# zoltanmaric/h264-fer

Hardware: AMD Instinct MI355X
Metric: macroblocks/sec encode (1080p full-search ME) + bit-exact bitstream vs ref (higher is better)
Workload: dtype u8; 1 GPU; 1080p IPPP encode, full-search +-16 ME (BASELINE configs[2]); content=textured, coded_size=1920x1072, streams_per_gpu=256, contexts_per_gpu=1, gop=30, qp=12, window=32, maxdiff=3, parallelism=1 x 256 independent closed-GOP streams

## Files before the change

h264-fer_amd/csrc/fer_me.hip:

```cpp
#include <stdlib.h>
#include "fer_internal.h"
#include "fer_mvpred.h"

#define INF_M 1000000000

struct WList {
    int m;
    int xy;
};

__device__ __forceinline__ int pack_xy(int x, int y) { return (x & 0xffff) | (y << 16); }
__device__ __forceinline__ int unp_x(int xy) { return (int)(short)(xy & 0xffff); }
__device__ __forceinline__ int unp_y(int xy) { return xy >> 16; }

__device__ __forceinline__ void wl_insert(WList &L, int K, int lane, bool valid, int m, int xy)
{
    int thr = lane_bcast(L.m, K - 1);
    unsigned long long mask = __ballot(valid && m < thr);
    while (mask) {
        int src = __ffsll((long long)mask) - 1;
        mask &= mask - 1;
        int cm = lane_bcast(m, src), cxy = lane_bcast(xy, src);
        int pos = __popcll(__ballot(lane < K && L.m <= cm));
        if (pos < K) {
// ... 164 lines not shown
    select_topk_ex<NB, true>(v, K, lane, sel, L, raw, fin, [&](int u) { return u * 64 + lane; });
}

typedef unsigned short u16x2_t __attribute__((ext_vector_type(2)));
typedef short i16x2_t __attribute__((ext_vector_type(2)));
__device__ __forceinline__ uint32_t pk_sub16(uint32_t a, uint32_t b)
{
    return __builtin_bit_cast(uint32_t, (u16x2_t)(__builtin_bit_cast(u16x2_t, a) - __builtin_bit_cast(u16x2_t, b)));
}
__device__ __forceinline__ uint32_t pk_abs16(uint32_t a)
{
    i16x2_t x = __builtin_bit_cast(i16x2_t, a), z = {0, 0};
    return __builtin_bit_cast(uint32_t, __builtin_elementwise_max(x, (i16x2_t)(z - x)));
}
struct SuPk {
    uint32_t s01, s23, s4;
    uint32_t d01, d23, d4;
    uint32_t s12, s34;
    uint32_t e12, e34;
};
__device__ __forceinline__ SuPk su_pack(const int s[5])
{
    SuPk p;
    p.s01 = (uint32_t)s[0] | ((uint32_t)s[1] << 16);
    p.s23 = (uint32_t)s[2] | ((uint32_t)s[3] << 16);
    p.s4 = (uint32_t)s[4];
    p.d01 = (uint32_t)(s[0] - s[1]) << 16;
    p.d23 = (uint32_t)(s[0] - s[2]) | ((uint32_t)(s[0] - s[3]) << 16);
    p.d4 = (uint32_t)(s[0] - s[4]);
    p.s12 = (uint32_t)s[1] | ((uint32_t)s[2] << 16);
    p.s34 = (uint32_t)s[3] | ((uint32_t)s[4] << 16);
    p.e12 = (uint32_t)(s[0] - s[1]) | ((uint32_t)(s[0] - s[2]) << 16);
    p.e34 = (uint32_t)(s[0] - s[3]) | ((uint32_t)(s[0] - s[4]) << 16);
    return p;
}
__device__ __forceinline__ int feat_dist_w(uint32_t a, uint32_t b, uint32_t c, const SuPk &p)
{
    uint32_t t = __builtin_amdgcn_sad_u16(a, p.s01, 0);
    t = __builtin_amdgcn_sad_u16(b, p.s23, t);
    t = __builtin_amdgcn_sad_u16(c, p.s4, t);
    uint32_t kk = __builtin_amdgcn_perm(a, a, 0x01000100);
    t = __builtin_amdgcn_sad_u16(pk_sub16(kk, a), p.d01, t);
    t = __builtin_amdgcn_sad_u16(pk_sub16(kk, b), p.d23, t);
    t = __builtin_amdgcn_sad_u16(pk_sub16(kk, c) & 0xffffu, p.d4, t);
    return (int)t;
}
__device__ __forceinline__ int feat_dist_rec(const uint16_t *__restrict__ rec, const SuPk &p)
{
    const uint32_t *r = (const uint32_t *)rec;
    return feat_dist_w(r[0], r[1], r[2], p);
}
struct FeatRec {
    uint32_t a, b, c;
};

__device__ __forceinline__ FeatRec feat_rec_direct(const IPlanes &ip, int W, int H, int frac, int refy, int refx)
{
    const int y = iclamp(refy, 0, H - 1), x = iclamp(refx, 0, W - 1);
    const uint8_t *p0 = ip.base + (size_t)frac * ip.plane + (size_t)y * ip.pitch + (x & ~3);
    const uint32_t sh = (uint32_t)(x & 3);
    uint32_t h84[8], hc[8];
#pragma unroll
    for (int r = 0; r < 8; r++) {
        const uint32_t *w = (const uint32_t *)(p0 + (size_t)r * ip.pitch);
        const uint32_t lo = __builtin_amdgcn_alignbyte(w[1], w[0], sh), hi = __builtin_amdgcn_alignbyte(w[2], w[1], sh);
        const uint32_t a4 = __builtin_amdgcn_sad_u8(lo, 0u, 0u);
        h84[r] = __builtin_amdgcn_sad_u8(hi, 0u, a4) | (a4 << 16);
        hc[r] = __builtin_amdgcn_udot4(hi, 0x00000101u, __builtin_amdgcn_udot4(lo, 0x00000101u, 0u, false), false);
    }
    const uint32_t top = h84[0] + h84[1] + h84[2] + h84[3], all = top + h84[4] + h84[5] + h84[6] + h84[7];
    const uint32_t k3 = (h84[0] + h84[1] + h84[4] + h84[5]) & 0xffffu;
    const uint32_t k4 = hc[0] + hc[1] + hc[2] + hc[3] + hc[4] + hc[5] + hc[6] + hc[7];
    FeatRec f;
    f.a = (all & 0xffffu) | (top << 16);
    f.b = (all >> 16) | (k3 << 16);
    f.c = k4;
    return f;
}

template <int R1>
struct LocalGeo {
    static constexpr int N1 = 2 * R1 + 1, PW = 2 * R1 + 8, NC = N1 * N1 * 16, NB = (NC + 63) / 64;
    static constexpr int HTAB = 8 * PW * N1 * 2;
};
template <int R1>
struct LocalLoads {
    static constexpr int ROUNDS = (8 * LocalGeo<R1>::PW + 63) / 64;
    uint4 w[2][ROUNDS];
};
template <int R1>
__device__ __forceinline__ void local_request(const IPlanes &ip, int W, int H, int px0, int py0, int lane, LocalLoads<R1> &ld)
{
    using G = LocalGeo<R1>;
    constexpr int N1 = G::N1, PW = G::PW;
#pragma unroll
    for (int half = 0; half < 2; half++)
#pragma unroll
        for (int k = 0; k < LocalLoads<R1>::ROUNDS; k++) ld.w[half][k] = make_uint4(0, 0, 0, 0);
    if (px0 + N1 - 1 < 0 || px0 >= W || py0 + N1 - 1 < 0 || py0 >= H) return;
    const uint8_t *mbase = ip.base - ((size_t)FER_IP_T * ip.pitch + FER_IP_L);
    const uint32_t obase = __umul24((uint32_t)(py0 + FER_IP_T), (uint32_t)ip.pitch) + (uint32_t)((px0 & ~3) + FER_IP_L);
#pragma unroll
    for (int half = 0; half < 2; half++) {
#pragma unroll
        for (int k = 0; k < LocalLoads<R1>::ROUNDS; k++) {
            const int tt = min(k * 64 + lane, 8 * PW - 1);
            const int fl = tt / PW, r = tt - fl * PW;
            typedef uint32_t u32x4_a4 __attribute__((ext_vector_type(4), aligned(4)));
            const u32x4_a4 v = *(const u32x4_a4 *)(mbase + (obase + __umul24((uint32_t)(half * 8 + fl), (uint32_t)ip.plane) + __umul24((uint32_t)r, (uint32_t)ip.pitch)));
            ld.w[half][k] = make_uint4(v.x, v.y, v.z, v.w);
        }
    }
}
template <int R1>
__device__ __forceinline__ void local_metrics(const IPlanes &ip, int W, int H, int px0, int py0, const SuPk &sp, int lane,
                                              uint32_t *htab, int *mtab, int half_lo = 0, int half_hi = 2, const LocalLoads<R1> *pre = nullptr)
{
    using G = LocalGeo<R1>;
    constexpr int N1 = G::N1, PW = G::PW;
    static_assert(PW + 3 <= 16, "the patch row must fit one 16-byte load");
    if (px0 + N1 - 1 < 0 || px0 >= W || py0 + N1 - 1 < 0 || py0 >= H) {
#pragma unroll
        for (int u = 0; u < G::NB; u++) mtab[u * 64 + lane] = -1;
        WAVE_LDS_SYNC();
        return;
    }
    const uint32_t sh = (uint32_t)(px0 & 3);
    const uint8_t *mbase = ip.base - ((size_t)FER_IP_T * ip.pitch + FER_IP_L);
    const uint32_t obase = __umul24((uint32_t)(py0 + FER_IP_T), (uint32_t)ip.pitch) + (uint32_t)((px0 & ~3) + FER_IP_L);
    for (int half = half_lo; half < half_hi; half++) {
#pragma unroll
        for (int t0 = 0; t0 < 8 * PW; t0 += 64) {
            const int t = t0 + lane;
            const int tt = min(t, 8 * PW - 1);
            const int fl = tt / PW, r = tt - fl * PW;
            typedef uint32_t u32x4_a4 __attribute__((ext_vector_type(4), aligned(4)));
            uint4 w;
            if (pre) {
                w = half == 0 ? pre->w[0][t0 / 64] : pre->w[1][t0 / 64];
            } else {
                const u32x4_a4 v = *(const u32x4_a4 *)(mbase + (obase + __umul24((uint32_t)(half * 8 + fl), (uint32_t)ip.plane) + __umul24((uint32_t)r, (uint32_t)ip.pitch)));
                w = make_uint4(v.x, v.y, v.z, v.w);
            }
            const uint32_t b0 = __builtin_amdgcn_alignbyte(w.y, w.x, sh), b1 = __builtin_amdgcn_alignbyte(w.z, w.y, sh),
                           b2 = __builtin_amdgcn_alignbyte(w.w, w.z, sh);
            if (t < 8 * PW) {
                uint32_t *o = htab + (size_t)tt * N1 * 2;
#pragma unroll
                for (int ix = 0; ix < N1; ix++) {
                    const uint32_t lo = ix < 4 ? __builtin_amdgcn_alignbyte(b1, b0, (uint32_t)(ix & 3)) : b1;
                    const uint32_t hi = ix < 4 ? __builtin_amdgcn_alignbyte(b2, b1, (uint32_t)(ix & 3)) : b2;
                    const uint32_t a4 = __builtin_amdgcn_sad_u8(lo, 0u, 0u);
                    o[ix * 2] = __builtin_amdgcn_sad_u8(hi, 0u, a4) | (a4 << 16);
                    o[ix * 2 + 1] = __builtin_amdgcn_udot4(hi, 0x00000101u, __builtin_amdgcn_udot4(lo, 0x00000101u, 0u, false), false);
                }
            }
        }
        WAVE_LDS_SYNC();
        if (lane < 8 * N1) {
            const int fl = lane / N1, ix = lane - fl * N1;
            uint32_t P84[PW + 1], Pc[PW + 1];
            P84[0] = 0;
            Pc[0] = 0;
#pragma unroll
            for (int r = 0; r < PW; r++) {
                const uint2 h = *(const uint2 *)(htab + ((size_t)(fl * PW + r) * N1 + ix) * 2);
                P84[r + 1] = P84[r] + h.x;
                Pc[r + 1] = Pc[r] + h.y;
            }
            const int refx = px0 + ix, wx = iabs(ix - R1) + 4;
            const bool xok = refx >= 0 && refx < W;
#pragma unroll
            for (int iy = 0; iy < N1; iy++) {
                const uint32_t all = P84[iy + 8] - P84[iy];
                const uint32_t k1 = (P84[iy + 4] - P84[iy]) & 0xffffu;
                const uint32_t k3 = ((P84[iy + 2] - P84[iy]) + (P84[iy + 6] - P84[iy + 4])) & 0xffffu;
                const uint32_t k4 = Pc[iy + 8] - Pc[iy];
                const int D = feat_dist_w((all & 0xffffu) | (k1 << 16), (all >> 16) | (k3 << 16), k4, sp);
                const int refy = py0 + iy;
                const int m = (int)__umul24((uint32_t)(wx + iabs(iy - R1)), (uint32_t)D) | ((xok && refy >= 0 && refy < H) ? 0 : -1);
                mtab[((ix * N1 + iy) << 4) + half * 8 + fl] = m;
            }
        }
        WAVE_LDS_SYNC();
    }
    if (half_lo == 0) {
#pragma unroll
        for (int c = G::NC + lane; c < G::NB * 64; c += 64) mtab[c] = -1;
    }
    WAVE_LDS_SYNC();
}

__device__ __forceinline__ FeatRec feat0_load(const uint16_t *__restrict__ F0, int W, int H, int refy, int refx)
{
    int y = iclamp(refy, 0, H - 1), x = iclamp(refx, 0, W - 1);
    const uint32_t *r = (const uint32_t *)((const char *)F0 + (__umul24((uint32_t)y, (uint32_t)W * 12u) + (uint32_t)x * 12u));
    FeatRec f;
    f.a = r[0];
    f.b = r[1];
    f.c = r[2];
    return f;
}

struct SrcBlk {
    uint32_t lo[8], hi[8];
};
__device__ __forceinline__ SrcBlk src_block_load(const uint8_t *__restrict__ Y, int W, int sx, int sy)
{
    SrcBlk b;
#pragma unroll
    for (int r = 0; r < 8; r++) {
        const uint32_t *q = (const uint32_t *)(Y + (size_t)(sy + r) * W + sx);
        b.lo[r] = __builtin_amdgcn_readfirstlane((int)q[0]);
        b.hi[r] = __builtin_amdgcn_readfirstlane((int)q[1]);
    }
    return b;
}
__device__ __forceinline__ int sad_lane(const IPlanes &ip, int W, int H, int sx, int sy, int mvx, int mvy, const SrcBlk &S)
{
    const int xPi = iclamp(sx + (mvx >> 2), 0, W - 1), yPi = iclamp(sy + (mvy >> 2), 0, H - 1);
    const uint32_t sh = (uint32_t)(xPi & 3);
    const uint32_t o0 = __umul24((uint32_t)((mvx & 3) + (mvy & 3) * 4), (uint32_t)ip.plane) + __umul24((uint32_t)yPi, (uint32_t)ip.pitch) + (uint32_t)(xPi & ~3);
    uint32_t w[8][3];
#pragma unroll
    for (int r = 0; r < 8; r++) {
        const uint32_t *a = (const uint32_t *)(ip.base + (o0 + __umul24((uint32_t)r, (uint32_t)ip.pitch)));
        w[r][0] = a[0];
        w[r][1] = a[1];
        w[r][2] = a[2];
    }
    uint32_t sad = 0;
#pragma unroll
    for (int r = 0; r < 8; r++) {
        const uint32_t r0 = __builtin_amdgcn_alignbyte(w[r][1], w[r][0], sh), r1 = __builtin_amdgcn_alignbyte(w[r][2], w[r][1], sh);
        sad = __builtin_amdgcn_sad_u8(r1, S.hi[r], __builtin_amdgcn_sad_u8(r0, S.lo[r], sad));
    }
    return (int)sad;
}

#define ME_WIDE_LDS 1156
#define ME_SEL_NB 25
#ifndef PRE_WAVES
#define PRE_WAVES 5
#endif
template <int WIN>
__global__ __launch_bounds__(64) __attribute__((amdgpu_waves_per_eu(PRE_WAVES, PRE_WAVES))) void k_me_pre(FerDev d)
{
    const int window = WIN ? WIN : d.window;
    __shared__ __attribute__((aligned(16))) int wide_m[ME_WIDE_LDS];
    __shared__ __attribute__((aligned(16))) int sel_lds[448];
    static_assert(LocalGeo<2>::HTAB <= ME_WIDE_LDS && LocalGeo<2>::NB * 64 <= 448, "LDS regions of k_me_pre");
    const int lane = threadIdx.x;
    const int s = blockIdx.y;
    if (d.hdr[s * 4 + 3] != 0) return;
    const unsigned bx = xcd_swizzle(blockIdx.x, gridDim.x);
    const int mb = (int)(bx >> 2), part = (int)(bx & 3);
    const int W = d.W, H = d.H;
    const size_t ysz = d.ysz;
    const uint8_t *Y = d.curY + (size_t)s * ysz;
    const IPlanes ip = ip_stream(d, s);
    const int sx = ((mb % d.mbw) << 4) + (part & 1) * 8, sy = ((mb / d.mbw) << 4) + (part >> 1) * 8;
    const size_t pidx = ((size_t)s * d.nmb + mb) * 4 + part;

#ifdef FER_PROBE
    const bool probe = FER_DBGF(d, 128) && s == 0 && (bx % 997) == 5;
    long long tmark = probe ? wall_clock64() : 0;
#define PP_MARK(k)                                                          \
    if (probe) {                                                            \
        long long now_ = wall_clock64();                                    \
        if (lane == 0) atomicAdd((unsigned long long *)&d.timing[32 + k], (unsigned long long)(now_ - tmark)); \
        tmark = now_;                                                       \
    }
#else
#define PP_MARK(k)
#endif
    constexpr int RRL = (WIN == 16) ? 1 : 2;
    LocalLoads<RRL> ld;
    const bool fast_path = (WIN == 32 || WIN == 16) && !FER_DBGF(d, 3) && !d.basic;
    if (fast_path) local_request<RRL>(ip, W, H, sx - RRL, sy - RRL, lane, ld);
    int px = lane & 7, py = lane >> 3;
    int v = Y[(size_t)(sy + py) * W + sx + px];
    int su[5];
    su[0] = wave_sum(v);
    su[1] = wave_sum(py > 3 ? 0 : v);
    su[2] = wave_sum(px > 3 ? 0 : v);
    su[3] = wave_sum((py & 3) > 1 ? 0 : v);
    su[4] = wave_sum((px & 3) > 1 ? 0 : v);
    if (lane < 5) d.suma[pidx * 5 + lane] = su[lane];
    if (d.basic) {
        if (lane == 0) {
            d.st3n[pidx] = 0;
            d.v0[pidx] = 0;
        }
        return;
    }
    const SuPk sp = su_pack(su);
    PP_MARK(0)

    WList L;
    L.m = INF_M;
    L.xy = 0;
    const int R = window / 2, n = 2 * R + 1;
    const int r2 = window / 16, n2w = 2 * r2 + 1, nloc = n2w * n2w * 16;
    const uint16_t *F0 = d.feat0 + (size_t)s * 6 * ysz;
    const int wb = (n * n + 63) >> 6;
    if ((WIN == 32 || WIN == 16) && !FER_DBGF(d, 3)) {
        constexpr int WCH = 6;
        constexpr int NN = (WIN ? WIN : 32) + 1;
        constexpr int NBc = WIN ? WIN : 32, RPB = 64 / NBc, NWB = (NN + RPB - 1) / RPB;
        constexpr int LB = LocalGeo<RRL>::NB;
        static_assert(LB <= 7, "ME_SEL_NB leaves room for 7 local batches");
        const int ix = lane % NBc, r0 = lane / NBc;
        const int rx = sx - R + ix;
        const bool xok = rx >= 0 && rx < W;
        const int wx = iabs(ix - R) + 4;
        const uint32_t colo = (uint32_t)iclamp(rx, 0, W - 1) * 12u, rowb = (uint32_t)W * 12u;
        auto fin = [&](int idx) {
            if (idx < wb * 64) return pack_xy((idx / n - R) * 4, (idx % n - R) * 4);
            int c = idx - wb * 64;
            int frac = c & 15, pos = c >> 4;
            return pack_xy((pos / n2w - r2) * 4 + (frac & 3), (pos % n2w - r2) * 4 + (frac >> 2));
        };
        uint32_t k0w[NWB];
#pragma unroll
        for (int b2 = 0; b2 < NWB; b2++) {
            const int ry = iclamp(sy - R + b2 * RPB + r0, 0, H - 1);
            k0w[b2] = *(const uint32_t *)((const char *)F0 + (colo + __umul24((uint32_t)ry, rowb)));
        }
        const uint32_t k0c = feat0_load(F0, W, H, sy - R + min(lane, NN - 1), sx + R).a;
        local_metrics<RRL>(ip, W, H, sx - r2, sy - r2, sp, lane, (uint32_t *)wide_m, sel_lds, 0, 2, &ld);
        int vloc[LB];
        unsigned lminl = 0xffffffffu;
#pragma unroll
        for (int u = 0; u < LB; u++) {
            vloc[u] = sel_lds[u * 64 + lane];
            lminl = min(lminl, (unsigned)vloc[u]);
        }
        int T = 0x7fffffff;
        if (__popcll(__ballot(lminl < (1u << 21))) >= 33) {
            int lo = 0, hi = (1 << 21) - 1;
            while (lo < hi) {
                const int mid = (lo + hi) >> 1;
                if (__popcll(__ballot(lminl <= (unsigned)mid)) >= 33)
                    hi = mid;
                else
                    lo = mid + 1;
            }
            T = lo;
        }
        int *surv = wide_m;
        int ns = 0;
        const uint32_t s0 = (uint32_t)su[0];
        bool done = false;
        if (T != 0x7fffffff) {
#pragma unroll
            for (int b2 = 0; b2 < NWB; b2++) {
                const int iy = b2 * RPB + r0;
                const int ry = sy - R + iy;
                const uint32_t lb = __umul24(5u * (uint32_t)(wx + iabs(iy - R)), __builtin_amdgcn_sad_u16(k0w[b2] & 0xffffu, s0, 0u));
                const bool take = xok && ry >= 0 && ry < H && iy < NN && lb <= (uint32_t)T;
                const unsigned long long mk = __ballot(take);
                if (mk) {
                    const int slot = ns + (int)__builtin_amdgcn_mbcnt_hi((uint32_t)(mk >> 32), __builtin_amdgcn_mbcnt_lo((uint32_t)mk, 0u));
                    if (take && slot < 128) surv[slot] = ix * NN + iy;
                    ns += __popcll(mk);
                }
            }
            {
                const int iy = lane, ry = sy - R + iy;
                const uint32_t lb = __umul24(5u * (uint32_t)(R + 4 + iabs(iy - R)), __builtin_amdgcn_sad_u16(k0c & 0xffffu, s0, 0u));
                const bool take = iy < NN && sx + R < W && ry >= 0 && ry < H && lb <= (uint32_t)T;
                const unsigned long long mk = __ballot(take);
                if (mk) {
                    const int slot = ns + (int)__builtin_amdgcn_mbcnt_hi((uint32_t)(mk >> 32), __builtin_amdgcn_mbcnt_lo((uint32_t)mk, 0u));
                    if (take && slot < 128) surv[slot] = (NN - 1) * NN + iy;
                    ns += __popcll(mk);
                }
            }
            WAVE_LDS_SYNC();
            if (ns <= 128) {
                int v[2 + LB], ar[2];
#pragma unroll
                for (int b2 = 0; b2 < 2; b2++) {
                    v[b2] = -1;
                    ar[b2] = 0;
                    if (b2 * 64 < ns) {
                        const int idx = b2 * 64 + lane;
                        const bool on = idx < ns;
                        const int ai = on ? surv[idx] : 0;
                        const int cix = ai / NN, ciy = ai - cix * NN;
                        const FeatRec f = feat0_load(F0, W, H, sy - R + ciy, sx - R + cix);
                        const int m = (int)__umul24((uint32_t)(iabs(cix - R) + iabs(ciy - R) + 4), (uint32_t)feat_dist_w(f.a, f.b, f.c, sp));
                        v[b2] = on ? m : -1;
                        ar[b2] = ai;
                    }
                }
#pragma unroll
                for (int u = 0; u < LB; u++) v[2 + u] = vloc[u];
                WAVE_LDS_SYNC();
                auto arrv = [&](int u) { return u < 2 ? ar[u < 2 ? u : 0] : wb * 64 + (u - 2) * 64 + lane; };
                done = select_topk_ex<2 + LB, false>(v, 33, lane, sel_lds, L, arrv, fin, arrv);
            }
        }
        PP_MARK(1)
#ifdef FER_STATS
        if (lane == 0) {
            atomicAdd((unsigned long long *)&d.timing[48], 1ull);
            atomicAdd((unsigned long long *)&d.timing[49], done ? 0ull : 1ull);
            atomicAdd((unsigned long long *)&d.timing[50], (unsigned long long)ns);
            atomicAdd((unsigned long long *)&d.timing[51], T == 0x7fffffff ? 1ull : 0ull);
            atomicAdd((unsigned long long *)&d.timing[52], (unsigned long long)(T == 0x7fffffff ? 0 : T));
        }
#endif
        if (!done) {
            WAVE_LDS_SYNC();
            auto wide_load = [&](int iy0, FeatRec (&fr)[WCH]) {
#pragma unroll
                for (int q = 0; q < WCH; q++) {
                    int ry = iclamp(sy - R + iy0 + q * RPB + r0, 0, H - 1);
                    const uint32_t *r = (const uint32_t *)((const char *)F0 + (colo + __umul24((uint32_t)ry, rowb)));
                    fr[q].a = r[0];
                    fr[q].b = r[1];
                    fr[q].c = r[2];
                }
            };
            auto wide_eval = [&](int iy0, const FeatRec (&fr)[WCH]) {
#pragma unroll
                for (int q = 0; q < WCH; q++) {
                    const int iy = iy0 + q * RPB + r0;
                    const int ry = sy - R + iy;
                    const int m = (int)__umul24((uint32_t)(wx + iabs(iy - R)), (uint32_t)feat_dist_w(fr[q].a, fr[q].b, fr[q].c, sp));
                    const int bad = (xok && ry >= 0 && ry < H) ? 0 : -1;
                    wide_m[iy < n ? ix * n + iy : ME_WIDE_LDS - 1] = m | bad;
                }
            };
            {
                constexpr int STEP = RPB * WCH;
                FeatRec fa[WCH], fb[WCH];
                wide_load(0, fa);
                for (int iy0 = 0; iy0 < n; iy0 += 2 * STEP) {
                    if (iy0 + STEP < n) wide_load(iy0 + STEP, fb);
                    wide_eval(iy0, fa);
                    if (iy0 + STEP < n) {
                        if (iy0 + 2 * STEP < n) wide_load(iy0 + 2 * STEP, fa);
                        wide_eval(iy0 + STEP, fb);
                    }
                }
            }
            {
                const int iy = min(lane, n - 1);
                const int rxl = sx + R, ry = sy - R + iy;
                FeatRec f = feat0_load(F0, W, H, ry, rxl);
                int m = (R + 4 + iabs(iy - R)) * feat_dist_w(f.a, f.b, f.c, sp);
                if (!(rxl < W && ry >= 0 && ry < H)) m = -1;
                if (lane < n) wide_m[(n - 1) * n + iy] = m;
            }
            __syncthreads();
            int v[ME_SEL_NB];
#pragma unroll
            for (int u = 0; u < ME_SEL_NB; u++) {
                v[u] = -1;
                if (u < wb) {
                    int c = u * 64 + lane;
                    if (c < n * n) v[u] = wide_m[c];
                } else if (u - wb < LB) {
                    v[u] = vloc[u - wb < LB ? u - wb : 0];
                }
            }
            WAVE_LDS_SYNC();
            auto raw = [&](int u) { return u * 64 + lane; };
            PP_MARK(2)
            select_topk<ME_SEL_NB>(v, 33, lane, sel_lds, L, raw, fin);
        }
        PP_MARK(3)
    } else {
        for (int base = 0; base < n * n && !FER_DBGF(d, 1); base += 64) {
            int c = base + lane;
            int tx = c / n - R, ty = c % n - R;
            int rx = sx + tx, ry = sy + ty;
            bool ok = c < n * n && rx >= 0 && rx < W && ry >= 0 && ry < H;
            int m = 0;
            if (ok) m = (iabs(tx) + iabs(ty) + 4) * feat_dist_rec(F0 + ((size_t)ry * W + rx) * 6, sp);
            wl_insert(L, 33, lane, ok, m, pack_xy(tx * 4, ty * 4));
        }
        for (int base = 0; base < nloc && !FER_DBGF(d, 2); base += 64) {
            int c = base + lane;
            int frac = c & 15, pos = c >> 4;
            int tx = pos / n2w - r2, ty = pos % n2w - r2;
            int rx = sx + tx, ry = sy + ty;
            bool ok = c < nloc && rx >= 0 && rx < W && ry >= 0 && ry < H;
            int m = 0;
            if (ok) {
                const FeatRec f = feat_rec_direct(ip, W, H, frac, ry, rx);
                m = (iabs(tx) + iabs(ty) + 4) * feat_dist_w(f.a, f.b, f.c, sp);
            }
            wl_insert(L, 33, lane, ok, m, pack_xy(tx * 4 + (frac & 3), ty * 4 + (frac >> 2)));
        }
    }
    const int n3 = __popcll(__ballot(lane < 33 && L.m < 100000000));
    int v0 = 0;
    if (!FER_DBGF(d, 4)) {
        const SrcBlk SB = src_block_load(Y, W, sx, sy);
        const int cx = unp_x(L.xy), cy = unp_y(L.xy);
        const int sad = sad_lane(ip, W, H, sx, sy, lane < n3 ? cx : 0, lane < n3 ? cy : 0, SB);
        if (lane < n3) {
            int *o = d.st3 + (pidx * 33 + lane) * 3;
            o[0] = cx;
            o[1] = cy;
            o[2] = sad;
        }
        const int wk = wave_min(lane < n3 ? (sad << 6) | lane : 0x7fffffff);
        if (wk != 0x7fffffff) v0 = lane_bcast(L.xy, wk & 63);
    }
    if (lane == 0) {
        d.st3n[pidx] = n3;
        d.v0[pidx] = v0;
    }

}

struct NoProbe {
    __device__ __forceinline__ int operator()(int) const { return 0; }
};
template <bool QUIRK, class SINK, class PROBE = NoProbe>
__device__ __forceinline__ int walk_buckets_q(const FerDev &d, int s, const int (&su)[5], const SuPk &sp, int sx, int sy, int lane,
                                              uint32_t *tbl, int halt_cnt, int &jend, SINK sink, uint32_t max_slice = 0xffffffffu,
                                              bool skip0 = false, PROBE probe = PROBE())
{
    int tren = 0;
    jend = 180;
    const int kt = d.kt;
    const uint32_t *kol2 = d.kol2 + (size_t)s * 16384 * kt;
    const uint32_t *srec = d.sort_rec;
    const int n0 = QUIRK ? d.zero_cnt[s] : 0;
    const uint32_t npos = (uint32_t)(d.W * d.H), g0 = (uint32_t)s * npos;
    const uint16_t *F0 = d.feat0 + (size_t)s * 6 * d.ysz;
    const int t_lo = QUIRK ? 0 : (max(sx - 279, 0) >> d.ktw_shift), t_hi = QUIRK ? kt - 1 : (min(sx + 279, d.W - 1) >> d.ktw_shift);
    auto qstart = [&](int a) -> uint32_t {
        if (a <= 0) return g0;
        if (a == 1) return g0 + min(2u * (uint32_t)n0, npos);
        if (a >= 16384) return g0 + npos;
        return kol2[(size_t)a * kt] - (uint32_t)n0;
    };
    const uint32_t sxy = ((uint32_t)sx << 16) | (uint32_t)sy;
    const char *srec_s = (const char *)(srec + (size_t)g0 * 3);
    auto fetch = [&](unsigned b_start, int b_cnt, uint32_t &r0, uint32_t &r1, uint32_t &r2) {
        const uint32_t li = (b_start - g0) + (unsigned)min(lane, max(b_cnt - 1, 0));
        const uint32_t *e = (const uint32_t *)(srec_s + __umul24(li, 12u));
        r0 = e[0];
        r1 = e[1];
        r2 = e[2];
    };
    auto passes = [&](uint32_t r0, uint32_t r1) -> bool {
        uint32_t dist = __builtin_amdgcn_sad_u16(r0, sxy, 0);
        uint32_t e12 = pk_abs16(pk_sub16(r1, sp.s12));
        return dist < 280u && (pk_sub16(e12, 0x00640064u) & 0x80008000u) == 0x80008000u;
    };
    auto feat_d = [&](uint32_t info, uint32_t r0, uint32_t r1, uint32_t r2) -> uint32_t {
        uint32_t D;
        if (!QUIRK) {
            const uint32_t aa = ((info >> 16) & 0x7fffu) * 0x10001u;
            D = __builtin_amdgcn_sad_u16(r1, sp.s12, (info >> 8) & 255u);
            D = __builtin_amdgcn_sad_u16(r2, sp.s34, D);
            D = __builtin_amdgcn_sad_u16(pk_sub16(aa, r1), sp.e12, D);
            D = __builtin_amdgcn_sad_u16(pk_sub16(aa, r2), sp.e34, D);
        } else {
            int px = min((int)(r0 >> 16), d.W - 1), py = min((int)(r0 & 0xffff), d.H - 1);
            D = (uint32_t)feat_dist_rec(F0 + ((size_t)py * d.W + px) * 6, sp);
        }
        return D;
    };
    auto filter = [&](uint32_t info, uint32_t r0, uint32_t r1, uint32_t r2) -> bool {
        const int b_cnt = (int)(info & 127u);
        bool ok = lane < b_cnt && passes(r0, r1);
        unsigned long long mk = __ballot(ok);
        int rank = tren + (int)__builtin_amdgcn_mbcnt_hi((uint32_t)(mk >> 32), __builtin_amdgcn_mbcnt_lo((uint32_t)mk, 0u));
        const uint32_t D = feat_d(info, r0, r1, r2);
        const bool halt = sink(ok, rank, (int)pk_sub16(r0, sxy), (int)D, info);
        tren += __popcll(mk);
        return halt || tren > halt_cnt;
    };
    auto run_table = [&](uint32_t dstart, uint32_t dinfo, int nb) -> bool {
        auto desc = [&](int b, unsigned &bs, uint32_t &bi) {
            const int bb = min(b, 63);
            bs = (unsigned)__builtin_amdgcn_readlane((int)dstart, bb);
            bi = (uint32_t)__builtin_amdgcn_readlane((int)dinfo, bb);
        };
        unsigned sA, sB, sC, sD;
        uint32_t iA, iB, iC, iD;
        uint32_t A0, A1, A2, B0, B1, B2, C0, C1, C2, D0, D1, D2;
        desc(0, sA, iA);
        fetch(sA, (int)(iA & 127u), A0, A1, A2);
        desc(1, sB, iB);
        fetch(sB, (int)(iB & 127u), B0, B1, B2);
        desc(2, sC, iC);
        fetch(sC, (int)(iC & 127u), C0, C1, C2);
        desc(3, sD, iD);
        fetch(sD, (int)(iD & 127u), D0, D1, D2);
#define WALK_STEP(SS, II, R0, R1, R2, NEXT)                                  \
        if (filter(II, R0, R1, R2)) {       \
            jend = (int)((II >> 8) & 255u);                                  \
// ... 713 lines not shown
    if (d.basic || FER_DBGF(d, 32)) return 0;
    const uint32_t cfl = (uint32_t)lane_bcast(P.e2[0].y, 41);
    const bool rewalk = (cfl & 0x40000000u) != 0 && ((cfl >> 16) & 15u) == 0;
    if (P.n2raw > FER_ST2_CAP && d.zero_cnt[s] == 0 && !rewalk) {
        resolve_crowded(d, s, sx, sy, lane, P, genx, geny, L2);
    } else if (P.n2raw > FER_ST2_CAP) {
        const SuPk sp = su_pack(P.su);
        int jx;
        walk_buckets(d, s, P.su, sp, sx, sy, lane, (uint32_t *)sel_lds, 0x7fffffff, jx, [&](bool ok, int rank, int rel, int D, uint32_t) {
            (void)rank;
            int tx = rel >> 16, ty = (int)(short)(rel & 0xffff);
            wl_insert(L2, 33, lane, ok, (iabs(tx - genx) + iabs(ty - geny) + 4) * D, pack_xy(tx * 4, ty * 4));
            return false;
        });
    } else {
        int m2[FER_ST2_CAP / 64];
#pragma unroll
        for (int u = 0; u < FER_ST2_CAP / 64; u++) {
            int cc = u * 64 + lane;
            int tx = P.e2[u].x >> 16, ty = (int)(short)(P.e2[u].x & 0xffff);
            m2[u] = (int)__umul24((uint32_t)(iabs(tx - genx) + iabs(ty - geny) + 4), (uint32_t)P.e2[u].y) | (cc < P.n2 ? 0 : -1);
        }
        auto raw2 = [&](int u) { return P.e2[u].x; };
        auto fin2 = [&](int e) { return pack_xy((e >> 16) * 4, (int)(short)(e & 0xffff) * 4); };
        select_topk<FER_ST2_CAP / 64>(m2, 33, lane, sel_lds, L2, raw2, fin2);
    }
    return __popcll(__ballot(lane < 33 && L2.m < 100000000));
}

template <int WIN>
__device__ __forceinline__ void resolve_stage23(const FerDev &d, int s, int gx, int gy, int lane, const ResPre &P, int mvpx, int mvpy,
                                                int *sel_lds, int &k2, int &xy2, int &k3, int &xy3)
{
    k2 = k3 = 0x7fffffff;
    xy2 = xy3 = 0;
    if (d.basic || FER_DBGF(d, 32)) return;
    WList L2;
    const int cnt2 = stage2_list(d, s, gx, gy, lane, P, mvpx >> 2, mvpy >> 2, sel_lds, L2);
    if (FER_DBGF(d, 256)) L2.xy = pack_xy(lane & 7, lane >> 3);
    int b2, b2xy;
    sad_keys<33>(L2, cnt2, lane, ip_stream(d, s), d.W, d.H, gx * 8, gy * 8, P.sb, mvpx, mvpy, b2, b2xy);
    wave_best(b2, b2xy, k2, xy2);
    int key = 0x7fffffff;
    if (lane < P.n3) key = ((P.c3s + iabs(P.c3x - mvpx) + iabs(P.c3y - mvpy)) << 6) | lane;
    wave_best(key, pack_xy(P.c3x, P.c3y), k3, xy3);
}

__device__ __forceinline__ ResNbr nbr_from_field(const FerDev &d, const int *vf, int gx, int gy, int lane)
{
    ResNbr N;
    nbr_avail(gx, gy, d.mbw * 2, N.vB, N.vC, N.vD, N.vC16);
    N.vA = gx > 0;
    const int xa = gx + (lane == 0 ? 0 : (lane == 1 ? 1 : (lane == 2 ? -1 : (lane == 3 ? 2 : -1)))), ya = lane == 4 ? gy : gy - 1;
    const bool val = lane == 0 ? N.vB : (lane == 1 ? N.vC : (lane == 2 ? N.vD : (lane == 3 ? N.vC16 : (lane == 4 && N.vA))));
    const int w = val ? vf[part_slot(d.mbw, xa, ya)] : 0;
    N.B = lane_bcast(w, 0);
    N.C = lane_bcast(w, 1);
    N.D = lane_bcast(w, 2);
    N.C16 = lane_bcast(w, 3);
    N.A = lane_bcast(w, 4);
    return N;
}

#ifndef SPEC_WAVES
#define SPEC_WAVES 7
#endif
template <int WIN>
__global__ __launch_bounds__(256) __attribute__((amdgpu_waves_per_eu(SPEC_WAVES, SPEC_WAVES))) void k_me_spec(FerDev d)
{
    __shared__ __attribute__((aligned(16))) uint32_t loc_all[4][LocalGeo<2>::HTAB + LocalGeo<2>::NB * 64];
    __shared__ int skipflag;
    static_assert(LocalGeo<2>::HTAB >= 256, "the selection's scratch fits the row sums");
    const int lane = threadIdx.x & 63;
    const int part = __builtin_amdgcn_readfirstlane(threadIdx.x >> 6);
    const int s = blockIdx.y;
    if (d.hdr[s * 4 + 3] != 0) return;
    const int mb = (int)xcd_swizzle(blockIdx.x, gridDim.x);
    const int mbx = mb % d.mbw, mby = mb / d.mbw;
    const int gx = mbx * 2 + (part & 1), gy = mby * 2 + (part >> 1);
    const size_t pidx = ((size_t)s * d.nmb + mb) * 4 + part;
    uint32_t *htab = loc_all[part];
    int *mtab = (int *)loc_all[part] + LocalGeo<2>::HTAB;
    int *sel_lds = (int *)loc_all[part];
    const ResNbr N = nbr_from_field(d, d.v0 + (size_t)s * d.nmb * 4, gx, gy, lane);
    int mvpx, mvpy;
    predict_nbr(N.vA, N.A, N.vB, N.B, N.vC, N.C, N.vD, N.D, mvpx, mvpy);
    const int genx = mvpx >> 2, geny = mvpy >> 2;
    const int genw = pack_xy(genx, geny);
    const int W = d.W, H = d.H;
    const IPlanes ip = ip_stream(d, s);
    const int sx = gx * 8, sy = gy * 8;
    constexpr int RRL = (WIN == 16) ? 1 : 2;
    LocalLoads<RRL> ld;
    if (WIN == 32 || WIN == 16) local_request<RRL>(ip, W, H, sx + genx - RRL, sy + geny - RRL, lane, ld);
    ResPre P;
    res_prefetch(d, s, gx, gy, lane, 1, P);
    int smw = 0;
    bool sk = false;
    if (part == 0) {
        int smx, smy;
        pskip_vector(d, mb, mbx, N, smx, smy);
        smw = pack_xy(smx, smy);
        sk = pskip_test(d, s, mbx, mby, lane, smx, smy);
        if (lane == 0) skipflag = sk;
    }
    __syncthreads();
    sk = skipflag != 0;
    if (sk) {
        if (lane == 0) d.spec_hdr[pidx] = make_int4(genw, part == 0 ? (1 << 17) : 0, smw, 1);
        return;
    }
    if (WIN == 32 || WIN == 16) local_metrics<RRL>(ip, W, H, sx + genx - RRL, sy + geny - RRL, su_pack(P.su), lane, htab, mtab, 0, 2, &ld);
    WList L1, L2;
    const int cnt1 = stage1_list<WIN>(d, s, gx, gy, lane, P, genx, geny, sel_lds, mtab, L1);
    const int cnt2 = stage2_list(d, s, gx, gy, lane, P, genx, geny, sel_lds, L2);
    {
        const int xy2 = __shfl(L2.xy, (lane - 17) & 63);
        const bool first = lane < 17;
        const int xy = first ? L1.xy : xy2;
        const bool on = first ? lane < cnt1 : (lane - 17 < cnt2 && lane < 50);
        const int cx = on ? unp_x(xy) : 0, cy = on ? unp_y(xy) : 0;
        const int sad = sad_lane(ip, W, H, sx, sy, cx, cy, P.sb);
        if (on) {
            int2 *o = first ? d.spec_l1 + (pidx * 17 + lane) : d.spec_l2 + (pidx * 33 + (lane - 17));
            *o = make_int2(xy, sad);
        }
    }
    if (lane == 0) d.spec_hdr[pidx] = make_int4(genw, cnt1 | (cnt2 << 8) | (1 << 16) | (part == 0 ? (1 << 17) : 0), smw, 0);
}

#ifndef RES_WIN
#define RES_WIN 16
#endif
#ifndef RES_WAVES
#define RES_WAVES 6
#endif
template <int WIN>
__global__ __launch_bounds__(64) __attribute__((amdgpu_waves_per_eu(RES_WAVES, RES_WAVES))) void k_me_resolve(FerDev d)
{
    __shared__ __attribute__((aligned(16))) uint32_t loc_lds[LocalGeo<2>::HTAB + LocalGeo<2>::NB * 64];
    const int lane = threadIdx.x;
    const int gw = d.mbw * 2, gh = d.mbh * 2;
    int xcc;
    asm volatile("s_getreg_b32 %0, hwreg(HW_REG_XCC_ID)" : "=s"(xcc));
    const int nq = d.S >= 16 ? 8 : 1;
    const int q_own = nq == 8 ? (xcc & 7) : 0;
    int q_done = 0;
    const bool spec = d.speculate != 0;
    unsigned st_parts = 0, st_hits = 0, st_skq = 0, st_skh = 0;
    for (;;) {
    const int qu = (q_own + q_done) & (nq - 1);
    const int nsq = (d.S - qu + nq - 1) / nq;
    int t = 0;
    if (lane == 0) t = atomicAdd(d.chain + qu, 1);
    t = __builtin_amdgcn_readfirstlane(t);
    const int G = min(d.resolve_group, nsq);
    const int grp = t / (gh * G), rr = t - grp * (gh * G);
    const int k0 = grp * G, kn = min(G, nsq - k0);
    if (k0 >= nsq) {
        if (++q_done == nq) break;
        continue;
    }
    const int gy = rr / kn, s = qu + nq * (k0 + (rr - gy * kn));
    if (gy >= gh) continue;
    if (d.hdr[s * 4 + 3] != 0) continue;
    unsigned long long *chw = d.chain64 + (size_t)s * d.nmb * 4;
    int *mbt = d.mb_type + (size_t)s * d.nmb;
    short *mvs = d.mv + (size_t)s * d.nmb * 8;
    const unsigned serial = (unsigned)d.serial & 0x7fffffffu;

#ifdef FER_PROBE
    const bool probe = FER_DBGF(d, 128) && s == 0 && gy == gh / 2;
#define PR_MARK(k)                        \
    if (probe) {                          \
        long long now_ = wall_clock64();  \
        tacc[k] += now_ - tmark;          \
        tmark = now_;                     \
    }
#else
    const bool probe = false;
#define PR_MARK(k)
#endif
    long long tacc[6] = {0, 0, 0, 0, 0, 0}, tmark = 0;
    int prevw = 0;
    bool skip = false, timeout = false;
    unsigned cwl = 0, cwh = 0;
    int wbase = 0;
    const size_t pidx0 = ((size_t)s * d.nmb + (size_t)(gy >> 1) * d.mbw) * 4 + (size_t)(gy & 1) * 2;
    const int4 *row_hdr = d.spec_hdr + pidx0;
    const int2 *row_l1 = d.spec_l1 + pidx0 * 17, *row_l2 = d.spec_l2 + pidx0 * 33;
    const int *row_st3 = d.st3 + pidx0 * 33 * 3, *row_st3n = d.st3n + pidx0;
    for (int gx = 0; gx < gw; gx++) {
        if (probe) tmark = wall_clock64();
        const int part = (gy & 1) * 2 + (gx & 1);
        const int mbx = gx >> 1, mby = gy >> 1;
        const int mb = mby * d.mbw + mbx;
        int ln = lane;
        asm volatile("" : "+v"(ln));
        int4 sh = make_int4(0, 0, 0, 0);
        int2 e1 = make_int2(0, 0), e2 = make_int2(0, 0);
        int c3x = 0, c3y = 0, c3s = 0, n3 = 0;
        if (spec) {
            const unsigned rp = (FER_DBGF(d, 512) ? 0u : (unsigned)((gx >> 1) * 4 + (gx & 1)));
            sh = row_hdr[rp];
            e1 = row_l1[rp * 17u + (unsigned)min(ln, 16)];
            e2 = row_l2[rp * 33u + (unsigned)min(ln, 32)];
            if (!d.basic) {
                const int *c3 = row_st3 + (rp * 33u + (unsigned)min(ln, 32)) * 3u;
                c3x = c3[0];
                c3y = c3[1];
                c3s = c3[2];
// ... 228 lines not shown
```

Before: 21.02 million macroblocks/s.

## Restructure local metric row loads into three shared rounds and drop prefix sums

Measured after the change: 21.35 million macroblocks/s, median of 6. 1.6% higher.

```diff
diff --git a/h264-fer_amd/csrc/fer_me.hip b/h264-fer_amd/csrc/fer_me.hip
--- a/h264-fer_amd/csrc/fer_me.hip
+++ b/h264-fer_amd/csrc/fer_me.hip
@@ -270,43 +270,44 @@
 struct LocalGeo {
     static constexpr int N1 = 2 * R1 + 1, PW = 2 * R1 + 8, NC = N1 * N1 * 16, NB = (NC + 63) / 64;
     static constexpr int HTAB = 8 * PW * N1 * 2;
+    static constexpr int HT = 8 * PW, ROUNDS = (2 * HT + 63) / 64;
 };
 template <int R1>
 struct LocalLoads {
-    static constexpr int ROUNDS = (8 * LocalGeo<R1>::PW + 63) / 64;
-    uint4 w[2][ROUNDS];
+    static constexpr int EARLY = LocalGeo<R1>::ROUNDS - 1;
+    uint4 w[EARLY];
 };
 template <int R1>
+__device__ __forceinline__ uint4 local_row_load(const uint8_t *mbase, uint32_t obase, const IPlanes &ip, int k, int lane)
+{
+    using G = LocalGeo<R1>;
+    const int t = min(k * 64 + lane, 2 * G::HT - 1);
+    const int fl = t / G::PW, r = t - fl * G::PW;
+    typedef uint32_t u32x4_a4 __attribute__((ext_vector_type(4), aligned(4)));
+    const u32x4_a4 v = *(const u32x4_a4 *)(mbase + (obase + __umul24((uint32_t)fl, (uint32_t)ip.plane) + __umul24((uint32_t)r, (uint32_t)ip.pitch)));
+    return make_uint4(v.x, v.y, v.z, v.w);
+}
+template <int R1>
 __device__ __forceinline__ void local_request(const IPlanes &ip, int W, int H, int px0, int py0, int lane, LocalLoads<R1> &ld)
 {
     using G = LocalGeo<R1>;
-    constexpr int N1 = G::N1, PW = G::PW;
-#pragma unroll
-    for (int half = 0; half < 2; half++)
-#pragma unroll
-        for (int k = 0; k < LocalLoads<R1>::ROUNDS; k++) ld.w[half][k] = make_uint4(0, 0, 0, 0);
+    constexpr int N1 = G::N1;
+#pragma unroll
+    for (int k = 0; k < LocalLoads<R1>::EARLY; k++) ld.w[k] = make_uint4(0, 0, 0, 0);
     if (px0 + N1 - 1 < 0 || px0 >= W || py0 + N1 - 1 < 0 || py0 >= H) return;
     const uint8_t *mbase = ip.base - ((size_t)FER_IP_T * ip.pitch + FER_IP_L);
     const uint32_t obase = __umul24((uint32_t)(py0 + FER_IP_T), (uint32_t)ip.pitch) + (uint32_t)((px0 & ~3) + FER_IP_L);
 #pragma unroll
-    for (int half = 0; half < 2; half++) {
-#pragma unroll
-        for (int k = 0; k < LocalLoads<R1>::ROUNDS; k++) {
-            const int tt = min(k * 64 + lane, 8 * PW - 1);
-            const int fl = tt / PW, r = tt - fl * PW;
-            typedef uint32_t u32x4_a4 __attribute__((ext_vector_type(4), aligned(4)));
-            const u32x4_a4 v = *(const u32x4_a4 *)(mbase + (obase + __umul24((uint32_t)(half * 8 + fl), (uint32_t)ip.plane) + __umul24((uint32_t)r, (uint32_t)ip.pitch)));
-            ld.w[half][k] = make_uint4(v.x, v.y, v.z, v.w);
-        }
-    }
+    for (int k = 0; k < LocalLoads<R1>::EARLY; k++) ld.w[k] = local_row_load<R1>(mbase, obase, ip, k, lane);
 }
 template <int R1>
 __device__ __forceinline__ void local_metrics(const IPlanes &ip, int W, int H, int px0, int py0, const SuPk &sp, int lane,
-                                              uint32_t *htab, int *mtab, int half_lo = 0, int half_hi = 2, const LocalLoads<R1> *pre = nullptr)
+                                              uint32_t *htab, int *mtab, const LocalLoads<R1> *pre = nullptr)
 {
     using G = LocalGeo<R1>;
-    constexpr int N1 = G::N1, PW = G::PW;
+    constexpr int N1 = G::N1, PW = G::PW, HT = G::HT, ROUNDS = G::ROUNDS;
     static_assert(PW + 3 <= 16, "the patch row must fit one 16-byte load");
+    static_assert(HT > 64 && HT <= 128 && ROUNDS == 3, "round 0 belongs to the first half, round 2 to the second, round 1 to both");
     if (px0 + N1 - 1 < 0 || px0 >= W || py0 + N1 - 1 < 0 || py0 >= H) {
 #pragma unroll
         for (int u = 0; u < G::NB; u++) mtab[u * 64 + lane] = -1;
@@ -316,66 +317,74 @@
     const uint32_t sh = (uint32_t)(px0 & 3);
     const uint8_t *mbase = ip.base - ((size_t)FER_IP_T * ip.pitch + FER_IP_L);
     const uint32_t obase = __umul24((uint32_t)(py0 + FER_IP_T), (uint32_t)ip.pitch) + (uint32_t)((px0 & ~3) + FER_IP_L);
-    for (int half = half_lo; half < half_hi; half++) {
-#pragma unroll
-        for (int t0 = 0; t0 < 8 * PW; t0 += 64) {
-            const int t = t0 + lane;
-            const int tt = min(t, 8 * PW - 1);
-            const int fl = tt / PW, r = tt - fl * PW;
-            typedef uint32_t u32x4_a4 __attribute__((ext_vector_type(4), aligned(4)));
-            uint4 w;
-            if (pre) {
-                w = half == 0 ? pre->w[0][t0 / 64] : pre->w[1][t0 / 64];
-            } else {
-                const u32x4_a4 v = *(const u32x4_a4 *)(mbase + (obase + __umul24((uint32_t)(half * 8 + fl), (uint32_t)ip.plane) + __umul24((uint32_t)r, (uint32_t)ip.pitch)));
-                w = make_uint4(v.x, v.y, v.z, v.w);
-            }
-            const uint32_t b0 = __builtin_amdgcn_alignbyte(w.y, w.x, sh), b1 = __builtin_amdgcn_alignbyte(w.z, w.y, sh),
-                           b2 = __builtin_amdgcn_alignbyte(w.w, w.z, sh);
-            if (t < 8 * PW) {
-                uint32_t *o = htab + (size_t)tt * N1 * 2;
-#pragma unroll
-                for (int ix = 0; ix < N1; ix++) {
-                    const uint32_t lo = ix < 4 ? __builtin_amdgcn_alignbyte(b1, b0, (uint32_t)(ix & 3)) : b1;
-                    const uint32_t hi = ix < 4 ? __builtin_amdgcn_alignbyte(b2, b1, (uint32_t)(ix & 3)) : b2;
-                    const uint32_t a4 = __builtin_amdgcn_sad_u8(lo, 0u, 0u);
-                    o[ix * 2] = __builtin_amdgcn_sad_u8(hi, 0u, a4) | (a4 << 16);
-                    o[ix * 2 + 1] = __builtin_amdgcn_udot4(hi, 0x00000101u, __builtin_amdgcn_udot4(lo, 0x00000101u, 0u, false), false);
-                }
-            }
-        }
-        WAVE_LDS_SYNC();
+    const uint4 wlast = local_row_load<R1>(mbase, obase, ip, ROUNDS - 1, lane);
+    auto row_sums = [&](int k, uint2 (&e)[N1]) {
+        const uint4 w = k == ROUNDS - 1 ? wlast : (pre ? pre->w[k] : local_row_load<R1>(mbase, obase, ip, k, lane));
+        const uint32_t b0 = __builtin_amdgcn_alignbyte(w.y, w.x, sh), b1 = __builtin_amdgcn_alignbyte(w.z, w.y, sh),
+                       b2 = __builtin_amdgcn_alignbyte(w.w, w.z, sh);
+#pragma unroll
+        for (int ix = 0; ix < N1; ix++) {
+            const uint32_t lo = ix < 4 ? __builtin_amdgcn_alignbyte(b1, b0, (uint32_t)(ix & 3)) : b1;
+            const uint32_t hi = ix < 4 ? __builtin_amdgcn_alignbyte(b2, b1, (uint32_t)(ix & 3)) : b2;
+            const uint32_t a4 = __builtin_amdgcn_sad_u8(lo, 0u, 0u);
+            e[ix].x = __builtin_amdgcn_sad_u8(hi, 0u, a4) | (a4 << 16);
+            e[ix].y = __builtin_amdgcn_udot4(hi, 0x00000101u, __builtin_amdgcn_udot4(lo, 0x00000101u, 0u, false), false);
+        }
+    };
+    auto row_store = [&](int tt, const uint2 (&e)[N1]) {
+        uint2 *o = (uint2 *)htab + tt * N1;
+#pragma unroll
+        for (int ix = 0; ix < N1; ix++) o[ix] = e[ix];
+    };
+    auto columns = [&](int half) {
         if (lane < 8 * N1) {
             const int fl = lane / N1, ix = lane - fl * N1;
-            uint32_t P84[PW + 1], Pc[PW + 1];
-            P84[0] = 0;
-            Pc[0] = 0;
+            uint32_t h84[PW], hc[PW];
 #pragma unroll
             for (int r = 0; r < PW; r++) {
                 const uint2 h = *(const uint2 *)(htab + ((size_t)(fl * PW + r) * N1 + ix) * 2);
-                P84[r + 1] = P84[r] + h.x;
-                Pc[r + 1] = Pc[r] + h.y;
-            }
+                h84[r] = h.x;
+                hc[r] = h.y;
+            }
+            uint32_t t2[PW - 1], u4[PW - 3];
+#pragma unroll
+            for (int r = 0; r < PW - 1; r++) t2[r] = h84[r] + h84[r + 1];
+#pragma unroll
+            for (int r = 0; r < PW - 3; r++) u4[r] = t2[r] + t2[r + 2];
+            uint32_t k4 = 0;
+#pragma unroll
+            for (int r = 0; r < 8; r++) k4 += hc[r];
             const int refx = px0 + ix, wx = iabs(ix - R1) + 4;
             const bool xok = refx >= 0 && refx < W;
 #pragma unroll
             for (int iy = 0; iy < N1; iy++) {
-                const uint32_t all = P84[iy + 8] - P84[iy];
-                const uint32_t k1 = (P84[iy + 4] - P84[iy]) & 0xffffu;
-                const uint32_t k3 = ((P84[iy + 2] - P84[iy]) + (P84[iy + 6] - P84[iy + 4])) & 0xffffu;
-                const uint32_t k4 = Pc[iy + 8] - Pc[iy];
+                const uint32_t all = u4[iy] + u4[iy + 4];
+                const uint32_t k1 = u4[iy] & 0xffffu;
+                const uint32_t k3 = (t2[iy] + t2[iy + 4]) & 0xffffu;
                 const int D = feat_dist_w((all & 0xffffu) | (k1 << 16), (all >> 16) | (k3 << 16), k4, sp);
                 const int refy = py0 + iy;
                 const int m = (int)__umul24((uint32_t)(wx + iabs(iy - R1)), (uint32_t)D) | ((xok && refy >= 0 && refy < H) ? 0 : -1);
                 mtab[((ix * N1 + iy) << 4) + half * 8 + fl] = m;
-            }
-        }
-        WAVE_LDS_SYNC();
-    }
-    if (half_lo == 0) {
-#pragma unroll
-        for (int c = G::NC + lane; c < G::NB * 64; c += 64) mtab[c] = -1;
-    }
+                if (iy + 1 < N1) k4 += hc[iy + 8] - hc[iy];
+            }
+        }
+    };
+    uint2 e[N1], held[N1];
+    row_sums(0, e);
+    row_store(lane, e);
+    row_sums(1, held);
+    const int t1 = 64 + lane;
+    if (t1 < HT) row_store(t1, held);
+    WAVE_LDS_SYNC();
+    columns(0);
+    WAVE_LDS_SYNC();
+    if (t1 >= HT) row_store(t1 - HT, held);
+    row_sums(2, e);
+    if (128 + lane < 2 * HT) row_store(128 + lane - HT, e);
+    WAVE_LDS_SYNC();
+    columns(1);
+#pragma unroll
+    for (int c = G::NC + lane; c < G::NB * 64; c += 64) mtab[c] = -1;
     WAVE_LDS_SYNC();
 }
 
@@ -516,7 +525,9 @@
             k0w[b2] = *(const uint32_t *)((const char *)F0 + (colo + __umul24((uint32_t)ry, rowb)));
         }
         const uint32_t k0c = feat0_load(F0, W, H, sy - R + min(lane, NN - 1), sx + R).a;
-        local_metrics<RRL>(ip, W, H, sx - r2, sy - r2, sp, lane, (uint32_t *)wide_m, sel_lds, 0, 2, &ld);
+        PP_MARK(1)
+        local_metrics<RRL>(ip, W, H, sx - r2, sy - r2, sp, lane, (uint32_t *)wide_m, sel_lds, &ld);
+        PP_MARK(2)
         int vloc[LB];
         unsigned lminl = 0xffffffffu;
 #pragma unroll
@@ -590,7 +601,7 @@
                 done = select_topk_ex<2 + LB, false>(v, 33, lane, sel_lds, L, arrv, fin, arrv);
             }
         }
-        PP_MARK(1)
+        PP_MARK(3)
 #ifdef FER_STATS
         if (lane == 0) {
             atomicAdd((unsigned long long *)&d.timing[48], 1ull);
@@ -657,10 +668,9 @@
             }
             WAVE_LDS_SYNC();
             auto raw = [&](int u) { return u * 64 + lane; };
-            PP_MARK(2)
             select_topk<ME_SEL_NB>(v, 33, lane, sel_lds, L, raw, fin);
         }
-        PP_MARK(3)
+        PP_MARK(4)
     } else {
         for (int base = 0; base < n * n && !FER_DBGF(d, 1); base += 64) {
             int c = base + lane;
@@ -704,7 +714,10 @@
         d.st3n[pidx] = n3;
         d.v0[pidx] = v0;
     }
-
+    PP_MARK(5)
+#ifdef FER_PROBE
+    if (probe && lane == 0) atomicAdd((unsigned long long *)&d.timing[39], 1ull);
+#endif
 }
 
 struct NoProbe {
@@ -1584,6 +1597,18 @@
     uint32_t *htab = loc_all[part];
     int *mtab = (int *)loc_all[part] + LocalGeo<2>::HTAB;
     int *sel_lds = (int *)loc_all[part];
+#ifdef FER_PROBE
+    const bool probe = FER_DBGF(d, 128) && s == 0 && (mb % 251) == 5;
+    long long tmark = probe ? wall_clock64() : 0;
+#define PS_MARK(k)                                                          \
+    if (probe) {                                                            \
+        long long now_ = wall_clock64();                                    \
+        if (lane == 0) atomicAdd((unsigned long long *)&d.timing[40 + k], (unsigned long long)(now_ - tmark)); \
+        tmark = now_;                                                       \
+    }
+#else
+#define PS_MARK(k)
+#endif
     const ResNbr N = nbr_from_field(d, d.v0 + (size_t)s * d.nmb * 4, gx, gy, lane);
     int mvpx, mvpy;
     predict_nbr(N.vA, N.A, N.vB, N.B, N.vC, N.C, N.vD, N.D, mvpx, mvpy);
@@ -1612,10 +1637,14 @@
         if (lane == 0) d.spec_hdr[pidx] = make_int4(genw, part == 0 ? (1 << 17) : 0, smw, 1);
         return;
     }
-    if (WIN == 32 || WIN == 16) local_metrics<RRL>(ip, W, H, sx + genx - RRL, sy + geny - RRL, su_pack(P.su), lane, htab, mtab, 0, 2, &ld);
+    PS_MARK(0)
+    if (WIN == 32 || WIN == 16) local_metrics<RRL>(ip, W, H, sx + genx - RRL, sy + geny - RRL, su_pack(P.su), lane, htab, mtab, &ld);
+    PS_MARK(1)
     WList L1, L2;
     const int cnt1 = stage1_list<WIN>(d, s, gx, gy, lane, P, genx, geny, sel_lds, mtab, L1);
+    PS_MARK(2)
     const int cnt2 = stage2_list(d, s, gx, gy, lane, P, genx, geny, sel_lds, L2);
+    PS_MARK(3)
     {
         const int xy2 = __shfl(L2.xy, (lane - 17) & 63);
         const bool first = lane < 17;
@@ -1629,6 +1658,10 @@
         }
     }
     if (lane == 0) d.spec_hdr[pidx] = make_int4(genw, cnt1 | (cnt2 << 8) | (1 << 16) | (part == 0 ? (1 << 17) : 0), smw, 0);
+    PS_MARK(4)
+#ifdef FER_PROBE
+    if (probe && lane == 0) atomicAdd((unsigned long long *)&d.timing[47], 1ull);
+#endif
 }
 
 #ifndef RES_WIN
```
